# naver/deep-image-retrieval

Hardware: AMD Instinct MI355X
Metric: images/sec descriptor extraction (resnet101-GeM, 1024x1024) (higher is better)
Workload: dtype fp16p

## Files before the change

### deep-image-retrieval_amd/csrc/engine.hip

```cpp
#include "engine.h"

#include <math.h>
#include <algorithm>

namespace dir {

static thread_local std::string g_err;
void set_error(const std::string& msg) { g_err = msg; }
int fail(int code, const std::string& msg) {
    g_err = msg;
    return code;
}
const char* last_error() { return g_err.c_str(); }


static Env read_env() {
    Env e;
    auto on = [](const char* k) { return getenv(k) != nullptr; };
    const char* mode = getenv("DIRTORCH_AMD_C3C1");
    e.c3c1_off = mode && mode[0] == '0';
    e.c3c1_force = mode && mode[0] == 'f';
    e.no_ds_seam = on("DIRTORCH_AMD_NO_DS_SEAM");
    e.no_dual = on("DIRTORCH_AMD_NO_DUAL");
    e.rev_conv1 = on("DIRTORCH_AMD_REV_CONV1");
// ... 379 lines not shown

int dir_engine::overflow(hipStream_t stream, int* overflowed) {
    if (!finalized) return fail(DIR_ERR_STATE, "overflow query before finalize");
    int host = 0;
    DIR_HIP_CHECK(hipMemcpyAsync(&host, d_ovf, sizeof(int), hipMemcpyDeviceToHost, stream));
    DIR_HIP_CHECK(hipMemsetAsync(d_ovf, 0, sizeof(int), stream));
    DIR_HIP_CHECK(hipStreamSynchronize(stream));
    *overflowed = host != 0;
    return DIR_OK;
}

static inline int conv_out(int h, int k, int stride, int pad) { return (h + 2 * pad - k) / stride + 1; }

int dir_engine::plan(int B, int H, int W, Plan* p) const {
    if (B <= 0 || H <= 0 || W <= 0) return fail(DIR_ERR_INVALID, "forward: B, H, W must be positive");
    if (H < 7 || W < 7) return fail(DIR_ERR_INVALID, "forward: image smaller than the 7x7 stem");
    p->H2 = (H + 1) / 2;
    p->W2 = (W + 1) / 2;
    p->OH1 = conv_out(H, 7, 2, 3);
    p->OW1 = conv_out(W, 7, 2, 3);
    p->PH = conv_out(p->OH1, 3, 2, 1);
    p->PW = conv_out(p->OW1, 3, 2, 1);
    const size_t es = dtype == DIR_F32 ? 4 : 2;
    size_t io = 0, t1 = 0, t2 = 0, ds = 0, x4 = 0;
    int h = p->PH, w = p->PW;
    io = (size_t)B * h * w * 64 * es;
    for (size_t bi = 0; bi < blocks.size(); ++bi) {
        const BlockDef& bd = blocks[bi];
        const int oh = conv_out(h, 3, bd.stride, 1), ow = conv_out(w, 3, bd.stride, 1);
        const ConvLayer& c1 = convs[bd.conv1];
        const ConvLayer& cl = convs[desc.bottleneck ? bd.conv3 : bd.conv2];
        if (desc.bottleneck) {
            t1 = std::max(t1, (size_t)B * h * w * c1.Cout * es);
            t2 = std::max(t2, (size_t)B * oh * ow * convs[bd.conv2].Cout * es);
        } else {
            t1 = std::max(t1, (size_t)B * oh * ow * c1.Cout * es);
        }
        if (bd.down >= 0) ds = std::max(ds, (size_t)B * oh * ow * convs[bd.down].Cout * es);
        io = std::max(io, (size_t)B * oh * ow * cl.Cout * es);
        h = oh;
        w = ow;
        if ((int)bi == x4_block) {
            x4 = (size_t)B * h * w * x4_dim * es;
            t2 = std::max(t2, x4);
        }
    }
    if (conv1x5 >= 0) t1 = std::max(t1, (size_t)B * h * w * x4_dim * es);
    size_t off = 0;
    auto take = [&](size_t bytes) {
        const size_t o = off;
        off += align_up(bytes);
        return o;
    };
    p->s2d = take((size_t)B * p->H2 * p->W2 * 16 * es);
    p->stem = take((size_t)B * p->OH1 * p->OW1 * 64 * es);
    p->bufA = take(io);
    p->bufB = take(io);
    p->t1 = take(t1);
    p->t2 = take(t2 ? t2 : 256);
    p->ds = take(ds ? ds : 256);
    p->x4 = take(x4 ? x4 : 256);
    p->lo_s2d = p->lo_stem = p->lo_t1 = p->lo_t2 = p->lo_ds = 0;
    if (dtype == DIR_FP16P) {
        size_t pt1 = 0, pt2 = 0, pds = 0;
        int ph = p->PH, pw = p->PW;
        for (int bi = 0; pair_acts && bi < pair_blocks && bi < (int)blocks.size(); ++bi) {
            const BlockDef& bd = blocks[bi];
            const int oh = conv_out(ph, 3, bd.stride, 1), ow = conv_out(pw, 3, bd.stride, 1);
            const ConvLayer& c1 = convs[bd.conv1];
            if (desc.bottleneck) {
                pt1 = std::max(pt1, (size_t)B * ph * pw * c1.Cout * 2);
                pt2 = std::max(pt2, (size_t)B * oh * ow * convs[bd.conv2].Cout * 2);
            } else {
                pt1 = std::max(pt1, (size_t)B * oh * ow * c1.Cout * 2);
            }
            if (bd.down >= 0) pds = std::max(pds, (size_t)B * oh * ow * convs[bd.down].Cout * 2);
            ph = oh;
            pw = ow;
        }
        p->lo_s2d = take((size_t)B * p->H2 * p->W2 * 16 * 2);
        p->lo_stem = take((size_t)B * p->PH * p->PW * 64 * 2);
        p->lo_t1 = take(pt1 ? pt1 : 256);
        p->lo_t2 = take(pt2 ? pt2 : 256);
        p->lo_ds = take(pds ? pds : 256);
    }
    p->splitk = take(kSplitKMaxBytes);
    p->pooled = take((size_t)B * head_dim * 4);
    p->fcout = take((size_t)B * std::max(desc.out_dim, head_dim) * 4);
    p->total = off;
    return DIR_OK;
}

int dir_engine::prof_begin(const std::string& name, const std::string& kernel, double flops,
                           double bytes, hipStream_t stream) {
    if (!profiling || prof_paused) return DIR_OK;
    if (prof_used == prof.size()) {
        ProfSlot s;
        DIR_HIP_CHECK(hipEventCreate(&s.start));
        DIR_HIP_CHECK(hipEventCreate(&s.stop));
        prof.push_back(s);
    }
    ProfSlot& s = prof[prof_used];
    s.name = name;
    s.kernel = kernel;
    s.flops = flops;
    s.bytes = bytes;
    DIR_HIP_CHECK(hipEventRecord(s.start, stream));
// ... 113 lines not shown
    a.x_lo = x_lo;
    a.w = L.d_w;
    a.w_lo = L.d_w_lo;
    a.bias = L.d_bias;
    a.res = res;
    a.res_lo = res_lo;
    a.y = y;
    a.y_lo = y_lo;
    a.B = B;
    a.H = H;
    a.W = W;
    a.OH = OH;
    a.OW = OW;
    a.Cin = L.Cin;
    a.Cout = L.Cout;
    a.R = L.R;
    a.S = L.S;
    a.stride = L.stride;
    a.pad = L.pad;
    a.relu = L.relu ? 1 : 0;
    a.ovf = d_ovf;
    a.M = B * OH * OW;
    a.Ktot = a.R * a.S * a.Cin;
    if (x2) {
        a.x2 = x2;
        a.x2_lo = x2_lo;
        a.Cin2 = a.Cin;
        a.w = L.d_w_ds;
        a.w_lo = L.d_w_ds_lo;
        a.bias = L.d_bias_ds;
        a.Ktot = 2 * a.Cin;
    }
    const double macs = (double)a.M * L.Cout * (double)a.Ktot;
    const double bytes = 2.0 * ((double)B * H * W * a.Cin * (x_lo ? 2 : 1) * (x2 ? 2 : 1) + (double)a.M * L.Cout * (y_lo ? 2 : 1) +
                                (double)a.M * L.Cout * (res ? (res_lo ? 2 : 1) : 0) + 2.0 * L.Cout * a.Ktot);
    int rc = DIR_OK;
    if (profiling && !prof_paused)
        rc = prof_begin(x2 ? L.name.substr(0, L.name.rfind('.')) + ".ds+conv3" : L.name,
                        std::string("conv_pair<") + conv_pair_variant_name(a) + ">", 2.0 * macs, bytes, stream);
    if (rc != DIR_OK) return rc;
    rc = conv_pair_launch(a, stream);
    if (rc != DIR_OK) return rc;
    return prof_end(stream);
}

int dir_engine::forward_pair_stem(const void* img, int B, int H, int W, int fmt, char* base, const Plan& p,
                                  hipStream_t stream) {
    uint16_t* s2d = (uint16_t*)(base + p.s2d);
    uint16_t* s2d_lo = (uint16_t*)(base + p.lo_s2d);
    int rc;
    if (img && fmt == DIR_IMG_U8_NHWC && d_stem_u8_w && !sw.no_stem_u8) {
        const bool raw = stem_pool_u8_raw_ok(img, B, H, W);
        if (!raw) {
            rc = prof_begin("prep_input", "prep_input_u8", 0, (double)B * H * W * 3 + (double)B * p.H2 * p.W2 * 32, stream);
            if (rc != DIR_OK) return rc;
            rc = prep_input_u8(img, s2d, B, H, W, stream);
            if (rc != DIR_OK) return rc;
            if ((rc = prof_end(stream)) != DIR_OK) return rc;
        }
        rc = prof_begin("conv1+maxpool", "stem_pool_u8", 2.0 * B * p.OH1 * p.OW1 * 64.0 * 147.0,
                        (raw ? (double)B * H * W * 3 : 2.0 * (double)B * p.H2 * p.W2 * 16) + 4.0 * ((double)B * p.PH * p.PW * 64 + 64 * 256),
                        stream);
        if (rc != DIR_OK) return rc;
        rc = stem_pool_u8_launch(raw ? img : nullptr, s2d, d_stem_u8_w, d_stem_u8_w_lo, d_stem_u8_bias, d_stem_u8_corr,
                                 (uint16_t*)(base + p.bufA), (uint16_t*)(base + p.lo_stem), B, H, W, stream, d_ovf, sw.stem_u8_seg);
        if (rc != DIR_OK) return rc;
        return prof_end(stream);
    }
    const bool raw_f32 = img && fmt == DIR_IMG_F32_NCHW && stem_pool_pair_raw_ok(img, B, H, W);
    if (img && !raw_f32) {
        rc = prof_begin("prep_input", "prep_input_pair", 0, (double)B * H * W * 3 * (fmt == DIR_IMG_U8_NHWC ? 1 : 4) +
                        (double)B * p.H2 * p.W2 * 64, stream);
        if (rc != DIR_OK) return rc;
        rc = prep_input_pair(img, fmt, desc.mean, desc.std, s2d, s2d_lo, B, H, W, stream);
        if (rc != DIR_OK) return rc;
        if ((rc = prof_end(stream)) != DIR_OK) return rc;
    } else if (!img) {
        const long n = (long)B * p.H2 * p.W2 * 16;
        hipLaunchKernelGGL(fill_noise_kernel, dim3((unsigned)((n + 255) / 256)), dim3(256), 0, stream, s2d, n, DIR_FP16);
        DIR_HIP_CHECK(hipGetLastError());
        DIR_HIP_CHECK(hipMemsetAsync(s2d_lo, 0, (size_t)n * 2, stream));
    }
    rc = prof_begin("conv1+maxpool", "stem_pool_pair", 2.0 * B * p.OH1 * p.OW1 * 64.0 * 147.0,
                    (raw_f32 ? (double)B * H * W * 12 : 4.0 * (double)B * p.H2 * p.W2 * 16) + 4.0 * ((double)B * p.PH * p.PW * 64 + 64 * 256), stream);
    if (rc != DIR_OK) return rc;
    if (raw_f32)
        rc = stem_pool_pair_walk_launch(nullptr, nullptr, convs[0].d_w, convs[0].d_w_lo, convs[0].d_bias, (uint16_t*)(base + p.bufA),
                                        (uint16_t*)(base + p.lo_stem), B, p.H2, p.W2, p.OH1, p.OW1, stream, d_ovf, img, H, W);
    else
        rc = stem_pool_pair_launch(s2d, s2d_lo, convs[0].d_w, convs[0].d_w_lo, convs[0].d_bias, (uint16_t*)(base + p.bufA),
                                   (uint16_t*)(base + p.lo_stem), B, p.H2, p.W2, p.OH1, p.OW1, stream, d_ovf);
    if (rc != DIR_OK) return rc;
    return prof_end(stream);
}

int dir_engine::forward_pair_head(const void* img, int B, int H, int W, int fmt, char* base, const Plan& p,
                                  hipStream_t stream, uint16_t** cur_out, int* h_out, int* w_out, size_t* next_block) {
    uint16_t* const pp[2] = {(uint16_t*)(base + p.bufA), (uint16_t*)(base + p.bufB)};
    uint16_t* stem_lo = (uint16_t*)(base + p.lo_stem);
    uint16_t* t1 = (uint16_t*)(base + p.t1);
    uint16_t* t2 = (uint16_t*)(base + p.t2);
    uint16_t* ds = (uint16_t*)(base + p.ds);
    uint16_t* t1_lo = (uint16_t*)(base + p.lo_t1);
    uint16_t* t2_lo = (uint16_t*)(base + p.lo_t2);
    uint16_t* ds_lo = (uint16_t*)(base + p.lo_ds);
    int rc = forward_pair_stem(img, B, H, W, fmt, base, p, stream);
    if (rc != DIR_OK) return rc;
    int cur = 0;

    int h = p.PH, w = p.PW;
    const size_t nb = std::min((size_t)pair_blocks, blocks.size());
    for (size_t bi = 0; bi < nb; ++bi) {
        BlockDef& bd = blocks[bi];
        const int oh = conv_out(h, 3, bd.stride, 1), ow = conv_out(w, 3, bd.stride, 1);
// ... 528 lines not shown
```

### deep-image-retrieval_amd/csrc/stem_u8.hip

```cpp
#include "dir_common.h"
#include "conv_igemm.h"
#include "pointwise.h"

#include <math.h>
#include <stdio.h>
#include <stdlib.h>
#include <vector>

#ifndef DIR_STEMU8_ABL
#define DIR_STEMU8_ABL 0
#endif

namespace dir {

static constexpr uint32_t kOOBu = 0x80000000u;

__device__ __forceinline__ void dma16u(__amdgpu_buffer_rsrc_t rsrc, char* lds, uint32_t voff) {
    __builtin_amdgcn_raw_ptr_buffer_load_lds(rsrc, (DIR_LDS void*)lds, 16, voff, 0, 0, 0);
}
__device__ __forceinline__ void split2u(float a, float b, uint32_t& hi, uint32_t& lo) {
    hi = FP16::pack(a, b);
    float ha, hb;
    FP16::unpack(hi, ha, hb);
    lo = FP16::pack(a - ha, b - hb);
// ... 14 lines not shown
    const float* bias;
    const float* corr;
    uint16_t *yh, *yl;
    int B, H, W, H2, W2, OH, OW, PH, PW;
    int tiles_x, nseg, seg_rows, nitems;
    uint32_t x_bytes;
    int* ovf;
};

struct TileU8 {
    int valid;
    int item, t, nt;
    int b, pw0;
    int pbase, pe;
    int c;
};

__device__ __forceinline__ int border_class(int o, int n) {
    const int t = 2 * o + 4 - n;
    return o == 0 ? 1 : (o == 1 ? 2 : (t <= 0 ? 0 : 2 + t));
}

template <int NRP, bool RAW, bool XPAIR = false>
__global__ void __launch_bounds__(128 * NRP, NRP == 2 ? 2 : 1) stem_pool_u8_kernel(const StemU8Args a) {
    typedef FP16 DT;
    typedef DT::frag_t frag_t;
    constexpr int PTW = 15;
    constexpr int NT = 128 * NRP;
    constexpr int TH = 2 * NRP, TW = 32;
    constexpr int QW = TW + 3;
    constexpr int QP = (TH + 3) * QW;
    constexpr int PLANE = NT * 16;
    constexpr int PATCH = (XPAIR ? 4 : 2) * PLANE;
    constexpr int NPB = XPAIR ? 2 : 3;
    constexpr int XROW = 16 * 256;
    constexpr int XBUF = 2 * NRP * XROW;
    static_assert(QP <= NT, "one DMA instruction per plane covers the patch");
    constexpr int X_OFF = NPB * PATCH;
    constexpr int BIAS_OFF = X_OFF + 2 * XBUF;
    constexpr int CORR_OFF = BIAS_OFF + 256;

    extern __shared__ __attribute__((aligned(16))) char smem[];

    const int tid = threadIdx.x;
    const int lane = tid & 63;
    const int wave = __builtin_amdgcn_readfirstlane(tid >> 6);
    const int lrow = lane & 31, lhi = lane >> 5;
    const int ci = wave & 1, rp = wave >> 1;

    const __amdgpu_buffer_rsrc_t rsrc_x = RAW ? __builtin_amdgcn_make_buffer_rsrc((void*)a.img, 0, a.img_bytes, 0x00020000)
                                              : __builtin_amdgcn_make_buffer_rsrc((void*)a.x, 0, a.x_bytes, 0x00020000);
    const __amdgpu_buffer_rsrc_t rsrc_xl = __builtin_amdgcn_make_buffer_rsrc((void*)(XPAIR ? a.xl : a.x), 0, a.x_bytes, 0x00020000);

    frag_t wfh[4][4], wfl[4][4];
#pragma unroll
    for (int R = 0; R < 4; ++R)
#pragma unroll
        for (int ks = 0; ks < 4; ++ks) {
            const size_t o = (size_t)(ci * 32 + lrow) * 256 + R * 64 + ks * 16 + lhi * 8;
            wfh[R][ks] = __builtin_bit_cast(frag_t, gload16(a.wh + o));
            wfl[R][ks] = __builtin_bit_cast(frag_t, gload16(a.wl + o));
        }
    float* lbias = (float*)(smem + BIAS_OFF);
    float* lcorr = (float*)(smem + CORR_OFF);
    if (tid < 64) lbias[tid] = a.bias[tid];
    if (!XPAIR)
        for (int i = tid; i < 36 * 64; i += NT) lcorr[i] = a.corr[i];

    auto decode = [&](TileU8& d) {
        d.valid = d.item < a.nitems;
        if (!d.valid) return;
        int r = d.item;
        const int tx = r % a.tiles_x;
        r /= a.tiles_x;
        d.b = r % a.B;
        const int seg = r / a.B;
        const int ps = seg * a.seg_rows;
        d.pe = min(a.PH, ps + a.seg_rows);
        d.nt = (2 * (d.pe - ps) + TH) / TH;
        d.pw0 = tx * PTW;
        d.pbase = ps + NRP * d.t;
        d.c = 2 * ps - 1 + TH * d.t;
    };
    auto advance = [&](TileU8& d) {
        if (!d.valid) return;
        if (++d.t < d.nt) {
            d.pbase += NRP;
            d.c += TH;
        } else {
            d.item += gridDim.x;
            d.t = 0;
            decode(d);
        }
    };
    const int ppy = tid / QW, ppx = tid - ppy * QW;
    const int ppoff = (ppy * a.W2 + ppx) * 32;
    auto issue_patch = [&](const TileU8& d, char* dst) {
        const int iy = d.c - 2 + ppy, ix = 2 * d.pw0 - 3 + ppx;
        const bool ok = tid < QP && (unsigned)iy < (unsigned)a.H2 && (unsigned)ix < (unsigned)a.W2;
        const int base = ((d.b * a.H2 + d.c - 2) * a.W2 + 2 * d.pw0 - 3) * 32;
        const uint32_t v = ok ? (uint32_t)(base + ppoff) : kOOBu;
        if (DIR_STEMU8_ABL & 4) return;
        dma16u(rsrc_x, dst + (wave * 64) * 16, v);
        dma16u(rsrc_x, dst + (NT + wave * 64) * 16, ok ? v + 16 : kOOBu);
        if (XPAIR) {
            dma16u(rsrc_xl, dst + (2 * NT + wave * 64) * 16, v);
            dma16u(rsrc_xl, dst + (3 * NT + wave * 64) * 16, ok ? v + 16 : kOOBu);
        }
    };

    uint32_t rw[XPAIR ? 12 : 6] = {};
    auto load_raw = [&](const TileU8& d) {
        const int iy = d.c - 2 + ppy, ix = 2 * d.pw0 - 3 + ppx;
        const bool ok = tid < QP && (unsigned)iy < (unsigned)a.H2 && (unsigned)ix < (unsigned)a.W2;
        if (XPAIR) {
            const int plane = a.H * a.W;
            const uint32_t o0 = ok ? (uint32_t)((((d.b * 3) * a.H + 2 * iy) * a.W + 2 * ix) * 4) : kOOBu;
            const bool row1 = ok && 2 * iy + 1 < a.H;
#pragma unroll
            for (int c = 0; c < 3; ++c)
#pragma unroll
                for (int dy = 0; dy < 2; ++dy) {
                    const uint32_t o = (dy == 0 ? ok : row1) ? o0 + (uint32_t)((c * plane + dy * a.W) * 4) : kOOBu;
                    const u32x2_t v = __builtin_bit_cast(u32x2_t, __builtin_amdgcn_raw_buffer_load_b64(rsrc_x, o, 0, 0));
                    rw[(c * 2 + dy) * 2] = v[0];
                    rw[(c * 2 + dy) * 2 + 1] = v[1];
                }
            return;
        }
        const uint32_t o0 = ok ? (uint32_t)(((d.b * a.H + 2 * iy) * a.W + 2 * ix) * 3) : kOOBu;
        const uint32_t o1 = (ok && 2 * iy + 1 < a.H) ? o0 + (uint32_t)(a.W * 3) : kOOBu;
#pragma unroll
        for (int k = 0; k < 3; ++k) {
            rw[k] = __builtin_amdgcn_raw_buffer_load_b16(rsrc_x, o0 + 2 * k, 0, 0);
            rw[3 + k] = __builtin_amdgcn_raw_buffer_load_b16(rsrc_x, o1 + 2 * k, 0, 0);
        }
    };
    auto store_raw = [&](char* dst) {
        if (XPAIR) {
            float f[12];
#pragma unroll
            for (int c = 0; c < 3; ++c)
#pragma unroll
                for (int dy = 0; dy < 2; ++dy)
#pragma unroll
                    for (int dx = 0; dx < 2; ++dx) f[(dy * 2 + dx) * 3 + c] = __builtin_bit_cast(float, rw[(c * 2 + dy) * 2 + dx]);
            u32x4_t h0, h1, l0, l1;
#pragma unroll
            for (int e = 0; e < 4; ++e) {
                uint32_t hh, ll;
                split2u(f[2 * e], f[2 * e + 1], hh, ll);
                h0[e] = hh;
                l0[e] = ll;
            }
#pragma unroll
            for (int e = 0; e < 2; ++e) {
                uint32_t hh, ll;
                split2u(f[8 + 2 * e], f[9 + 2 * e], hh, ll);
                h1[e] = hh;
                l1[e] = ll;
            }
            h1[2] = h1[3] = l1[2] = l1[3] = 0;
            *(u32x4_t*)(dst + tid * 16) = h0;
            *(u32x4_t*)(dst + (NT + tid) * 16) = h1;
            *(u32x4_t*)(dst + (2 * NT + tid) * 16) = l0;
            *(u32x4_t*)(dst + (3 * NT + tid) * 16) = l1;
            return;
        }
        float f[12];
#pragma unroll
        for (int k = 0; k < 6; ++k) {
            f[2 * k] = (float)(rw[k] & 0xffu) * 0.00390625f;
            f[2 * k + 1] = (float)((rw[k] >> 8) & 0xffu) * 0.00390625f;
        }
        u32x4_t p0, p1;
#pragma unroll
        for (int e = 0; e < 4; ++e) p0[e] = FP16::pack(f[2 * e], f[2 * e + 1]);
        p1[0] = FP16::pack(f[8], f[9]);
        p1[1] = FP16::pack(f[10], f[11]);
        p1[2] = p1[3] = 0;
        *(u32x4_t*)(dst + tid * 16) = p0;
        *(u32x4_t*)(dst + (NT + tid) * 16) = p1;
    };

    TileU8 cur, nxt, pre, prev;
    cur.item = blockIdx.x;
    cur.t = 0;
    decode(cur);
    if (!cur.valid) return;
    nxt = cur;
    advance(nxt);
    pre = nxt;
    advance(pre);
    prev.valid = 0;
    prev.t = prev.b = prev.pw0 = prev.pbase = prev.pe = 0;

    Ovf<DT> ovf;
    asm volatile("s_waitcnt vmcnt(0) lgkmcnt(0)" ::: "memory");
#pragma unroll
    for (int R = 0; R < 4; ++R)
#pragma unroll
        for (int ks = 0; ks < 4; ++ks) {
            asm volatile("" : "+v"(wfh[R][ks]));
            asm volatile("" : "+v"(wfl[R][ks]));
        }
    if (RAW) {
        load_raw(cur);
        store_raw(smem);
        if (nxt.valid) load_raw(nxt);
    } else {
        issue_patch(cur, smem);
        if (!XPAIR && nxt.valid) issue_patch(nxt, smem + PATCH);
    }

    int pb = 0;
    int xb = 0;
    for (;;) {
        if (RAW)
            asm volatile("s_waitcnt lgkmcnt(0)" ::: "memory");
        else if (XPAIR)
            asm volatile("s_waitcnt vmcnt(0) lgkmcnt(0)" ::: "memory");
        else if (nxt.valid)
            asm volatile("s_waitcnt vmcnt(2) lgkmcnt(0)" ::: "memory");
        else
            asm volatile("s_waitcnt vmcnt(0) lgkmcnt(0)" ::: "memory");
        ring_barrier();

        if (RAW) {
            if (nxt.valid) store_raw(smem + (pb == NPB - 1 ? 0 : pb + 1) * PATCH);
            if (pre.valid) load_raw(pre);
        } else if (XPAIR) {
            if (nxt.valid) issue_patch(nxt, smem + (pb ^ 1) * PATCH);
        } else if (pre.valid) {
            const int nb = pb == 0 ? 2 : pb - 1;
            issue_patch(pre, smem + nb * PATCH);
        }

        if (prev.valid && !(DIR_STEMU8_ABL & 2)) {
            const char* X = smem + X_OFF + (xb ^ 1) * XBUF;
            const int r4 = tid >> 7, px = (tid >> 3) & 15, c8 = tid & 7;
            const int ph = r4 < NRP - 1 ? prev.pbase + r4 : prev.pbase - 1;
            const int pw = prev.pw0 + px;
            const bool live = px < PTW && pw < a.PW && ph < prev.pe && (r4 < NRP - 1 || prev.t > 0);
            if (live) {
                const int o0 = px * 256 + (((2 * c8) ^ (px & 7)) << 4), o1 = px * 256 + (((2 * c8 + 1) ^ (px & 7)) << 4);
                f32x4_t m0, m1;
                if (r4 < NRP - 1) {
                    const f32x4_t a0 = *(const f32x4_t*)(X + r4 * XROW + o0), a1 = *(const f32x4_t*)(X + r4 * XROW + o1);
                    const f32x4_t b0 = *(const f32x4_t*)(X + (NRP + r4) * XROW + o0), b1 = *(const f32x4_t*)(X + (NRP + r4) * XROW + o1);
#pragma unroll
                    for (int e = 0; e < 4; ++e) {
                        m0[e] = fmaxf(a0[e], b0[e]);
                        m1[e] = fmaxf(a1[e], b1[e]);
                    }
                } else {
                    m0 = *(const f32x4_t*)(X + (2 * NRP - 1) * XROW + o0);
                    m1 = *(const f32x4_t*)(X + (2 * NRP - 1) * XROW + o1);
                }
                f32x4_t bb0 = {0.f, 0.f, 0.f, 0.f}, bb1 = {0.f, 0.f, 0.f, 0.f};
                if (!XPAIR) {
                    bb0 = *(const f32x4_t*)(lbias + c8 * 8);
                    bb1 = *(const f32x4_t*)(lbias + c8 * 8 + 4);
                }
                u32x4_t oh, ol;
                float mv[8];
#pragma unroll
                for (int e = 0; e < 4; ++e) {
                    mv[e] = fmaxf(XPAIR ? m0[e] : m0[e] + bb0[e], 0.f);
                    mv[4 + e] = fmaxf(XPAIR ? m1[e] : m1[e] + bb1[e], 0.f);
                }
#pragma unroll
                for (int e = 0; e < 4; ++e) {
                    uint32_t hh, ll;
                    split2u(mv[2 * e], mv[2 * e + 1], hh, ll);
                    oh[e] = hh;
                    ol[e] = ll;
                }
                const size_t o = ((size_t)(prev.b * a.PH + ph) * a.PW + pw) * 64 + c8 * 8;
                gstore16(a.yh + o, oh);
                gstore16(a.yl + o, ol);
                ovf.see(oh);
            }
        }
        if (!cur.valid) break;

        const char* pbuf = smem + pb * PATCH;
        const int ox = 2 * cur.pw0 - 1 + lrow;
        const int oy = cur.c + 2 * rp;
        const bool edge = cur.c <= 1 || 2 * (cur.c + TH - 1) + 4 > a.H || cur.pw0 == 0 || 2 * (2 * cur.pw0 + TW - 2) + 4 > a.W;
        f32x16_t acc[2];
        if (XPAIR) {
#pragma unroll
            for (int g = 0; g < 4; ++g) {
                const f32x4_t b4 = *(const f32x4_t*)(lbias + ci * 32 + 8 * g + 4 * lhi);
#pragma unroll
                for (int j = 0; j < 2; ++j)
#pragma unroll
                    for (int e = 0; e < 4; ++e) acc[j][4 * g + e] = b4[e];
            }
        } else {
#pragma unroll
            for (int j = 0; j < 2; ++j)
#pragma unroll
                for (int e = 0; e < 16; ++e) acc[j][e] = 0.f;
        }
        const char* xrow = pbuf + lhi * PLANE + ((rp * 2) * QW + lrow) * 16;
        frag_t xf[2], xg[2];
        xf[0] = *(const frag_t*)xrow;
        if (XPAIR) xg[0] = *(const frag_t*)(xrow + 2 * PLANE);
#pragma unroll
        for (int s = 0; s < 20; ++s) {
            const int q = s >> 2, ks = s & 3;
            if (s + 1 < 20) {
                xf[(s + 1) & 1] = *(const frag_t*)(xrow + (((s + 1) >> 2) * QW + ((s + 1) & 3)) * 16);
                if (XPAIR) xg[(s + 1) & 1] = *(const frag_t*)(xrow + 2 * PLANE + (((s + 1) >> 2) * QW + ((s + 1) & 3)) * 16);
            }
            if (!(DIR_STEMU8_ABL & 1)) {
                if (q < 4) {
                    acc[0] = DT::mfma32(wfh[q][ks], xf[s & 1], acc[0]);
                    if (XPAIR) acc[0] = DT::mfma32(wfh[q][ks], xg[s & 1], acc[0]);
                    acc[0] = DT::mfma32(wfl[q][ks], xf[s & 1], acc[0]);
                }
                if (q > 0) {
                    acc[1] = DT::mfma32(wfh[q - 1][ks], xf[s & 1], acc[1]);
                    if (XPAIR) acc[1] = DT::mfma32(wfh[q - 1][ks], xg[s & 1], acc[1]);
                    acc[1] = DT::mfma32(wfl[q - 1][ks], xf[s & 1], acc[1]);
                }
            }
            if (XPAIR) continue;
            __builtin_amdgcn_sched_group_barrier(0x100, 1, 0);
            if (q > 0 && q < 4)
                __builtin_amdgcn_sched_group_barrier(0x008, 4, 0);
            else
                __builtin_amdgcn_sched_group_barrier(0x008, 2, 0);
        }

        if (edge) {
            const bool col_in = (unsigned)ox < (unsigned)a.OW;
            const int cc = XPAIR ? 0 : border_class(min(max(ox, 0), a.OW - 1), a.W);
#pragma unroll
            for (int j = 0; j < 2; ++j) {
                const bool in = col_in && (unsigned)(oy + j) < (unsigned)a.OH;
                const int rc = XPAIR ? 0 : border_class(min(max(oy + j, 0), a.OH - 1), a.H);
#pragma unroll
                for (int g = 0; g < 4; ++g) {
                    f32x4_t c4 = {0.f, 0.f, 0.f, 0.f};
                    if (!XPAIR) c4 = *(const f32x4_t*)(lcorr + (rc * 6 + cc) * 64 + ci * 32 + 8 * g + 4 * lhi);
#pragma unroll
                    for (int e = 0; e < 4; ++e) {
                        const float t = acc[j][4 * g + e];
                        acc[j][4 * g + e] = in ? t + c4[e] : -__builtin_inff();
                    }
                }
            }
        }
#pragma unroll
        for (int j = 0; j < 2; ++j)
#pragma unroll
            for (int e = 0; e < 16; ++e) {
                const float v = acc[j][e];
                acc[j][e] = fmaxf(fmaxf(lane_left(v), v), lane_right(v));
            }
        char* X = smem + X_OFF + xb * XBUF;
        const int px = lrow >> 1;
        const bool odd = (lrow & 1) != 0;
        if (rp == 0 && cur.t > 0) {
            const char* Xp = smem + X_OFF + (xb ^ 1) * XBUF;
            if (odd) {
#pragma unroll
                for (int g = 0; g < 4; ++g) {
                    const int off = px * 256 + (((8 * ci + 2 * g + lhi) ^ (px & 7)) << 4);
                    const f32x4_t m3 = *(const f32x4_t*)(Xp + (NRP - 1) * XROW + off);
                    f32x4_t v;
#pragma unroll
                    for (int e = 0; e < 4; ++e) v[e] = fmaxf(m3[e], acc[0][4 * g + e]);
                    *(f32x4_t*)(X + (2 * NRP - 1) * XROW + off) = v;
                }
            }
        }
        if (odd) {
#pragma unroll
            for (int g = 0; g < 4; ++g) {
                const int off = px * 256 + (((8 * ci + 2 * g + lhi) ^ (px & 7)) << 4);
                f32x4_t h, m;
#pragma unroll
                for (int e = 0; e < 4; ++e) {
                    h[e] = acc[0][4 * g + e];
                    m[e] = fmaxf(acc[0][4 * g + e], acc[1][4 * g + e]);
                }
                *(f32x4_t*)(X + rp * XROW + off) = m;
                if (rp > 0) *(f32x4_t*)(X + (NRP - 1 + rp) * XROW + off) = h;
            }
        }

        prev = cur;
        cur = nxt;
        nxt = pre;
        advance(pre);
        pb = pb == NPB - 1 ? 0 : pb + 1;
        xb ^= 1;
    }
    ovf.flush(a.ovf);
}

__global__ void __launch_bounds__(256) prep_input_u8_kernel(const uint8_t* __restrict__ img, uint16_t* __restrict__ out, int B, int H,
                                                            int W, int H2, int W2) {
    const long idx = (long)blockIdx.x * blockDim.x + threadIdx.x;
    const long total = (long)B * H2 * W2;
    if (idx >= total) return;
    const int x2 = (int)(idx % W2);
    const int y2 = (int)((idx / W2) % H2);
    const int b = (int)(idx / ((long)W2 * H2));
    float v[16];
#pragma unroll
    for (int e = 0; e < 16; ++e) v[e] = 0.f;
#pragma unroll
    for (int dy = 0; dy < 2; ++dy) {
        const int y = 2 * y2 + dy;
        if (y >= H) continue;
        const uint8_t* row = img + (((size_t)b * H + y) * W + 2 * x2) * 3;
        const int n = (2 * x2 + 1 < W) ? 6 : 3;
#pragma unroll
        for (int k = 0; k < 6; ++k)
            if (k < n) v[dy * 6 + k] = (float)row[k] * 0.00390625f;
    }
    u32x4_t o0, o1;
#pragma unroll
    for (int e = 0; e < 4; ++e) {
        o0[e] = FP16::pack(v[2 * e], v[2 * e + 1]);
        o1[e] = FP16::pack(v[8 + 2 * e], v[8 + 2 * e + 1]);
    }
    gstore16(out + idx * 16, o0);
    gstore16(out + idx * 16 + 8, o1);
}

int fold_stem_u8(const float* w, const float* scale, const float* bias, const float* mean3, const float* std3,
                 std::vector<uint16_t>& hi, std::vector<uint16_t>& lo, std::vector<float>& b2, std::vector<float>& corr) {
    for (int c = 0; c < 3; ++c)
        if (!(std3[c] > 0.f)) return fail(DIR_ERR_INVALID, "stem_u8: preprocess std must be positive");
    const int lo_r[6] = {0, 3, 1, 0, 0, 0}, hi_r[6] = {6, 6, 6, 5, 4, 3};
    std::vector<float> packed((size_t)64 * 256, 0.f);
    b2.assign(64, 0.f);
    corr.assign((size_t)36 * 64, 0.f);
    for (int o = 0; o < 64; ++o) {
        double all = 0.0;
        double in[6][6];
        for (int rc = 0; rc < 6; ++rc)
            for (int cc = 0; cc < 6; ++cc) in[rc][cc] = 0.0;
        for (int c = 0; c < 3; ++c) {
            const double ms = (double)mean3[c] / (double)std3[c];
            for (int r = 0; r < 7; ++r)
                for (int s = 0; s < 7; ++s) {
                    const double ws = (double)w[(((size_t)o * 3 + c) * 7 + r) * 7 + s] * (double)scale[o];
                    all += ws * ms;
                    for (int rc = 0; rc < 6; ++rc)
                        for (int cc = 0; cc < 6; ++cc)
                            if (r >= lo_r[rc] && r <= hi_r[rc] && s >= lo_r[cc] && s <= hi_r[cc]) in[rc][cc] += ws * ms;
                    const int R = (r + 1) >> 1, dy = (r + 1) & 1, S = (s + 1) >> 1, dx = (s + 1) & 1;
                    packed[(((size_t)o * 4 + R) * 4 + S) * 16 + (dy * 2 + dx) * 3 + c] = (float)(ws * 256.0 / (255.0 * (double)std3[c]));
                }
        }
        b2[o] = (float)((double)bias[o] - all);
        for (int rc = 0; rc < 6; ++rc)
            for (int cc = 0; cc < 6; ++cc) corr[((size_t)rc * 6 + cc) * 64 + o] = (float)(all - in[rc][cc]);
    }
    hi.resize(packed.size());
    lo.resize(packed.size());
    for (size_t i = 0; i < packed.size(); ++i) {
        hi[i] = f32_to_f16_bits(packed[i]);
        if ((hi[i] & 0x7c00u) == 0x7c00u && std::isfinite(packed[i]))
            return fail(DIR_ERR_RANGE, "finalize: a BatchNorm-folded weight of conv1, folded with the image normalisation (" + std::to_string(packed[i]) +
                                           ") exceeds the fp16 range; use DIR_BF16 or DIR_F32");
        lo[i] = f32_to_f16_bits(packed[i] - f16_bits_to_f32(hi[i]));
    }
    return DIR_OK;
}

int prep_input_u8(const void* img, void* out, int B, int H, int W, hipStream_t stream) {
    if (!img || !out) return fail(DIR_ERR_INVALID, "prep_input_u8: null pointer");
    const int H2 = (H + 1) / 2, W2 = (W + 1) / 2;
    const long total = (long)B * H2 * W2;
    hipLaunchKernelGGL(prep_input_u8_kernel, dim3((unsigned)((total + 255) / 256)), dim3(256), 0, stream, (const uint8_t*)img,
                       (uint16_t*)out, B, H, W, H2, W2);
    DIR_HIP_CHECK(hipGetLastError());
    return DIR_OK;
}

bool stem_pool_u8_raw_ok(const void* img, int B, int H, int W) {
    return img && (W % 2) == 0 && ((uintptr_t)img & 1) == 0 && (size_t)B * H * W * 3 < (1ull << 31) && !env().stem_u8_prep &&
           !env().stem_u8_wg8;
}

int stem_pool_u8_launch(const void* img, const void* s2d, const void* w_hi, const void* w_lo, const float* bias, const float* corr,
                        void* y_hi, void* y_lo, int B, int H, int W, hipStream_t stream, int* ovf, int seg_tiles) {
    const bool raw = stem_pool_u8_raw_ok(img, B, H, W);
    if ((!raw && !s2d) || !w_hi || !w_lo || !bias || !corr || !y_hi || !y_lo) return fail(DIR_ERR_INVALID, "stem_pool_u8: null pointer");
    if (H < 7 || W < 7) return fail(DIR_ERR_INVALID, "stem_pool_u8: image smaller than the 7x7 stem");
    StemU8Args a;
    a.img = (const uint8_t*)img;
    a.img_bytes = raw ? (uint32_t)((size_t)B * H * W * 3) : 0;
    a.x = (const uint16_t*)s2d;
    a.xl = nullptr;
    a.wh = (const uint16_t*)w_hi;
    a.wl = (const uint16_t*)w_lo;
    a.bias = bias;
    a.corr = corr;
    a.yh = (uint16_t*)y_hi;
    a.yl = (uint16_t*)y_lo;
    a.B = B; a.H = H; a.W = W;
    a.H2 = (H + 1) / 2;
    a.W2 = (W + 1) / 2;
    a.OH = (H - 1) / 2 + 1;
    a.OW = (W - 1) / 2 + 1;
    a.PH = (a.OH - 1) / 2 + 1;
    a.PW = (a.OW - 1) / 2 + 1;
    if (!raw && (size_t)B * a.H2 * a.W2 * 32 >= (1ull << 31))
        return fail(DIR_ERR_INVALID, "stem_pool_u8: input exceeds 2^31 bytes; lower the batch");
    a.x_bytes = raw ? 0 : (uint32_t)((size_t)B * a.H2 * a.W2 * 32);
    a.tiles_x = (a.PW + 14) / 15;
    const bool wg8 = env().stem_u8_wg8;
    const int cus = cu_count();
    const int slots = wg8 ? cus : 2 * cus;
    int T = seg_tiles > 0 ? seg_tiles : 8;
    while (seg_tiles <= 0 && T > 1 && (long)B * a.tiles_x * ((a.PH + 4 * T - 2) / (4 * T - 1)) < 2L * slots) T >>= 1;
    a.seg_rows = 4 * T - 1;
    a.nseg = (a.PH + a.seg_rows - 1) / a.seg_rows;
    a.nitems = B * a.tiles_x * a.nseg;
    a.ovf = ovf;
    const int grid = a.nitems < slots ? a.nitems : slots;
    if (wg8) {
        constexpr int LDS = 3 * 16384 + 2 * 8 * 4096 + 256 + 36 * 64 * 4;
        static std::atomic<uint64_t> attr{0};
        DIR_HIP_CHECK(ensure_dynamic_lds((const void*)(stem_pool_u8_kernel<4, false>), LDS, attr));
        hipLaunchKernelGGL((stem_pool_u8_kernel<4, false>), dim3((unsigned)grid), dim3(512), LDS, stream, a);
    } else {
        constexpr int LDS = 3 * 8192 + 2 * 4 * 4096 + 256 + 36 * 64 * 4;
        static std::atomic<uint64_t> attr{0};
        static std::atomic<uint64_t> attr_raw{0};
        DIR_HIP_CHECK(ensure_dynamic_lds((const void*)(stem_pool_u8_kernel<2, false>), LDS, attr));
        DIR_HIP_CHECK(ensure_dynamic_lds((const void*)(stem_pool_u8_kernel<2, true>), LDS, attr_raw));
        static const bool dbg = getenv("DIRTORCH_AMD_DEBUG_OCCUPANCY") != nullptr;
        static std::atomic<int> told{0};
        if (dbg && !told.exchange(1)) {
            int nb = -1;
            (void)hipOccupancyMaxActiveBlocksPerMultiprocessor(&nb, (const void*)(stem_pool_u8_kernel<2, true>), 256, LDS);
            fprintf(stderr, "stem_pool_u8_kernel<2>: %d workgroups of 256 threads per CU at %d bytes of LDS (grid %d, %d items)\n", nb, LDS, grid,
                    a.nitems);
        }
        if (raw)
            hipLaunchKernelGGL((stem_pool_u8_kernel<2, true>), dim3((unsigned)grid), dim3(256), LDS, stream, a);
        else
            hipLaunchKernelGGL((stem_pool_u8_kernel<2, false>), dim3((unsigned)grid), dim3(256), LDS, stream, a);
    }
    DIR_HIP_CHECK(hipGetLastError());
    return DIR_OK;
}

bool stem_pool_pair_raw_ok(const void* img_f32, int B, int H, int W) {
    return img_f32 && (W % 2) == 0 && ((uintptr_t)img_f32 & 7) == 0 && (size_t)B * 3 * H * W * 4 < (1ull << 31) && !env().stem_u8_prep &&
           !env().stem_pair_old && !env().stem_v1;
}

int stem_pool_pair_walk_launch(const void* s2d_hi, const void* s2d_lo, const void* w_hi, const void* w_lo, const float* bias,
                               void* y_hi, void* y_lo, int B, int H2, int W2, int OH, int OW, hipStream_t stream, int* ovf,
                               const void* img_f32, int H, int W) {
    const bool raw = stem_pool_pair_raw_ok(img_f32, B, H, W);
    if ((!raw && (!s2d_hi || !s2d_lo)) || !w_hi || !w_lo || !bias || !y_hi || !y_lo) return fail(DIR_ERR_INVALID, "stem_pool_pair: null pointer");
    if (!raw && (size_t)B * H2 * W2 * 32 >= (1ull << 31)) return fail(DIR_ERR_INVALID, "stem_pool_pair: input exceeds 2^31 bytes; lower the batch");
    StemU8Args a;
    a.img = (const uint8_t*)(raw ? img_f32 : nullptr);
    a.img_bytes = raw ? (uint32_t)((size_t)B * 3 * H * W * 4) : 0;
// ... 39 lines not shown
```

### deep-image-retrieval_amd/dirtorch_amd/ops.py

```python
import ctypes

import torch

from . import _lib
from ._lib import DIR_BF16, DIR_FP16, POOLING, call, ptr, stream_ptr


def _dtype_code(t):
    if t.dtype == torch.bfloat16:
        return DIR_BF16
    if t.dtype == torch.float16:
        return DIR_FP16
    raise TypeError('16-bit activation tensor expected (bfloat16 or float16), got %s' % t.dtype)


def _need_cuda(*ts):
    for t in ts:
        if t is not None and not t.is_cuda:
            raise ValueError('device tensor expected')
        if t is not None and not t.is_contiguous():
            raise ValueError('contiguous tensor expected')


def conv_variant_names():
# ... 331 lines not shown
    y_hi = torch.empty(B, H, W, Cout, dtype=torch.float16, device=t_hi.device)
    y_lo = torch.empty_like(y_hi) if pair_out else None
    call('dir_conv_pair_dual', ptr(t_hi), ptr(t_lo), ptr(x_hi), ptr(x_lo), ptr(w_hi), ptr(w_lo), ptr(bias), ptr(y_hi),
         ptr(y_lo), B, H, W, Cin, Cout, int(bool(relu)), stream_ptr())
    return y_hi, y_lo


def prep_input_pair(img, mean=None, std=None):
    _need_cuda(img)
    if img.dtype == torch.float32:
        B, C, H, W = img.shape
        fmt = _lib.DIR_IMG_F32_NCHW
    elif img.dtype == torch.uint8:
        B, H, W, C = img.shape
        fmt = _lib.DIR_IMG_U8_NHWC
    else:
        raise TypeError('image must be float32 NCHW or uint8 NHWC')
    if C != 3:
        raise ValueError('3-channel image expected')
    hi = torch.empty(B, (H + 1) // 2, (W + 1) // 2, 16, dtype=torch.float16, device=img.device)
    lo = torch.empty_like(hi)
    m = (ctypes.c_float * 3)(*(mean or (0, 0, 0)))
    s = (ctypes.c_float * 3)(*(std or (1, 1, 1)))
    call('dir_prep_input_pair', ptr(img), fmt, m, s, ptr(hi), ptr(lo), B, H, W, stream_ptr())
    return hi, lo


def stem_pool_pair(s2d, w_packed, bias, out_hw):
    (s_hi, s_lo), (w_hi, w_lo) = s2d, w_packed
    _need_cuda(s_hi, s_lo, w_hi, w_lo, bias)
    B, H2, W2, _ = s_hi.shape
    OH, OW = out_hw
    PH, PW = (OH - 1) // 2 + 1, (OW - 1) // 2 + 1
    y_hi = torch.empty(B, PH, PW, 64, dtype=torch.float16, device=s_hi.device)
    y_lo = torch.empty_like(y_hi)
    call('dir_stem_pool_pair', ptr(s_hi), ptr(s_lo), ptr(w_hi), ptr(w_lo), ptr(bias), ptr(y_hi), ptr(y_lo), B, H2, W2,
         OH, OW, stream_ptr())
    return y_hi, y_lo


def stem_pool_u8(img_u8, w_oihw, bn_scale, bn_bias, mean, std, seg_tiles=0):
    _need_cuda(img_u8)
    if img_u8.dtype != torch.uint8 or img_u8.dim() != 4 or img_u8.shape[3] != 3:
        raise TypeError('image must be uint8 NHWC [B,H,W,3]')
    B, H, W, _ = img_u8.shape
    OH, OW = (H - 1) // 2 + 1, (W - 1) // 2 + 1
    PH, PW = (OH - 1) // 2 + 1, (OW - 1) // 2 + 1
    w = w_oihw.detach().to('cpu', torch.float32).contiguous()
    sc = bn_scale.detach().to('cpu', torch.float32).contiguous()
    bi = bn_bias.detach().to('cpu', torch.float32).contiguous()
    assert tuple(w.shape) == (64, 3, 7, 7) and sc.numel() == 64 and bi.numel() == 64
    m = (ctypes.c_float * 3)(*mean)
    s = (ctypes.c_float * 3)(*std)
    ws = torch.empty(B * ((H + 1) // 2) * ((W + 1) // 2) * 32, dtype=torch.uint8, device=img_u8.device)
    y_hi = torch.empty(B, PH, PW, 64, dtype=torch.float16, device=img_u8.device)
    y_lo = torch.empty_like(y_hi)
    call('dir_stem_pool_u8', ptr(img_u8.contiguous()), ctypes.c_void_p(w.data_ptr()), ctypes.c_void_p(sc.data_ptr()),
         ctypes.c_void_p(bi.data_ptr()), m, s, ptr(ws), ptr(y_hi), ptr(y_lo), B, H, W, int(seg_tiles), stream_ptr())
    return y_hi, y_lo


def pca_whiten(X, components, mean=None, alpha=None, l2norm=False, eps_unused=None, unit_range=False):
    _need_cuda(X, components, mean, alpha)
    for t in (X, components, mean, alpha):
        if t is not None and (t.dtype != torch.float32 or not t.is_contiguous()):
            raise TypeError('contiguous float32 tensors expected')
    N, D = X.shape
    v, D2 = components.shape
    if D != D2:
        raise ValueError('inner dimensions differ')
    out = torch.empty(N, v, dtype=torch.float32, device=X.device)
    if N == 0:
        return out
    call('dir_pca_whiten_l2_unit' if unit_range else 'dir_pca_whiten_l2', ptr(X), N, D, ptr(mean), ptr(components), v, ptr(alpha),
         int(bool(l2norm)), ptr(out), stream_ptr())
    return out
```

Baseline: 2467.

## Repack u8 stem input so conv1 K-dimension uses three MFMA slices instead of four

The space-to-depth layout for the uint8 stem now packs the 12 real channels per 2x2 cell so that the 7x7 conv reduction uses three 16-wide K slices per row instead of four zero-padded ones. The input buffer gains one extra padded column, the prep kernel and raw loader write shifted/overlapping halves, and the weight packing is reorganised to match. This cuts MFMA count and weight registers in the stem by about a quarter, at the cost of more complex indexing, a slightly larger staging buffer and extra LDS writes in the raw path.

```diff
diff --git a/deep-image-retrieval_amd/csrc/engine.hip b/deep-image-retrieval_amd/csrc/engine.hip
--- a/deep-image-retrieval_amd/csrc/engine.hip
+++ b/deep-image-retrieval_amd/csrc/engine.hip
@@ -455,7 +455,7 @@
         off += align_up(bytes);
         return o;
     };
-    p->s2d = take((size_t)B * p->H2 * p->W2 * 16 * es);
+    p->s2d = take((size_t)B * p->H2 * (p->W2 + (dtype == DIR_FP16P ? 1 : 0)) * 16 * es);
     p->stem = take((size_t)B * p->OH1 * p->OW1 * 64 * es);
     p->bufA = take(io);
     p->bufB = take(io);
@@ -675,14 +675,14 @@
     if (img && fmt == DIR_IMG_U8_NHWC && d_stem_u8_w && !sw.no_stem_u8) {
         const bool raw = stem_pool_u8_raw_ok(img, B, H, W);
         if (!raw) {
-            rc = prof_begin("prep_input", "prep_input_u8", 0, (double)B * H * W * 3 + (double)B * p.H2 * p.W2 * 32, stream);
+            rc = prof_begin("prep_input", "prep_input_u8", 0, (double)B * H * W * 3 + (double)B * p.H2 * (p.W2 + 1) * 32, stream);
             if (rc != DIR_OK) return rc;
             rc = prep_input_u8(img, s2d, B, H, W, stream);
             if (rc != DIR_OK) return rc;
             if ((rc = prof_end(stream)) != DIR_OK) return rc;
         }
         rc = prof_begin("conv1+maxpool", "stem_pool_u8", 2.0 * B * p.OH1 * p.OW1 * 64.0 * 147.0,
-                        (raw ? (double)B * H * W * 3 : 2.0 * (double)B * p.H2 * p.W2 * 16) + 4.0 * ((double)B * p.PH * p.PW * 64 + 64 * 256),
+                        (raw ? (double)B * H * W * 3 : 2.0 * (double)B * p.H2 * (p.W2 + 1) * 16) + 4.0 * ((double)B * p.PH * p.PW * 64 + 64 * 192),
                         stream);
         if (rc != DIR_OK) return rc;
         rc = stem_pool_u8_launch(raw ? img : nullptr, s2d, d_stem_u8_w, d_stem_u8_w_lo, d_stem_u8_bias, d_stem_u8_corr,
diff --git a/deep-image-retrieval_amd/csrc/stem_u8.hip b/deep-image-retrieval_amd/csrc/stem_u8.hip
--- a/deep-image-retrieval_amd/csrc/stem_u8.hip
+++ b/deep-image-retrieval_amd/csrc/stem_u8.hip
@@ -90,12 +90,13 @@
                                               : __builtin_amdgcn_make_buffer_rsrc((void*)a.x, 0, a.x_bytes, 0x00020000);
     const __amdgpu_buffer_rsrc_t rsrc_xl = __builtin_amdgcn_make_buffer_rsrc((void*)(XPAIR ? a.xl : a.x), 0, a.x_bytes, 0x00020000);
 
-    frag_t wfh[4][4], wfl[4][4];
+    constexpr int KS = XPAIR ? 4 : 3;
+    frag_t wfh[4][KS], wfl[4][KS];
 #pragma unroll
     for (int R = 0; R < 4; ++R)
 #pragma unroll
-        for (int ks = 0; ks < 4; ++ks) {
-            const size_t o = (size_t)(ci * 32 + lrow) * 256 + R * 64 + ks * 16 + lhi * 8;
+        for (int ks = 0; ks < KS; ++ks) {
+            const size_t o = (size_t)(ci * 32 + lrow) * (64 * KS) + R * (16 * KS) + ks * 16 + lhi * 8;
             wfh[R][ks] = __builtin_bit_cast(frag_t, gload16(a.wh + o));
             wfl[R][ks] = __builtin_bit_cast(frag_t, gload16(a.wl + o));
         }
@@ -132,11 +133,12 @@
         }
     };
     const int ppy = tid / QW, ppx = tid - ppy * QW;
-    const int ppoff = (ppy * a.W2 + ppx) * 32;
+    const int xw = XPAIR ? a.W2 : a.W2 + 1, xs = XPAIR ? 0 : 1;
+    const int ppoff = (ppy * xw + ppx) * 32;
     auto issue_patch = [&](const TileU8& d, char* dst) {
         const int iy = d.c - 2 + ppy, ix = 2 * d.pw0 - 3 + ppx;
-        const bool ok = tid < QP && (unsigned)iy < (unsigned)a.H2 && (unsigned)ix < (unsigned)a.W2;
-        const int base = ((d.b * a.H2 + d.c - 2) * a.W2 + 2 * d.pw0 - 3) * 32;
+        const bool ok = tid < QP && (unsigned)iy < (unsigned)a.H2 && (unsigned)(ix + xs) < (unsigned)xw;
+        const int base = ((d.b * a.H2 + d.c - 2) * xw + 2 * d.pw0 - 3 + xs) * 32;
         const uint32_t v = ok ? (uint32_t)(base + ppoff) : kOOBu;
         if (DIR_STEMU8_ABL & 4) return;
         dma16u(rsrc_x, dst + (wave * 64) * 16, v);
@@ -151,6 +153,7 @@
     auto load_raw = [&](const TileU8& d) {
         const int iy = d.c - 2 + ppy, ix = 2 * d.pw0 - 3 + ppx;
         const bool ok = tid < QP && (unsigned)iy < (unsigned)a.H2 && (unsigned)ix < (unsigned)a.W2;
+        if (DIR_STEMU8_ABL & 4) return;
         if (XPAIR) {
             const int plane = a.H * a.W;
             const uint32_t o0 = ok ? (uint32_t)((((d.b * 3) * a.H + 2 * iy) * a.W + 2 * ix) * 4) : kOOBu;
@@ -211,14 +214,15 @@
             f[2 * k] = (float)(rw[k] & 0xffu) * 0.00390625f;
             f[2 * k + 1] = (float)((rw[k] >> 8) & 0xffu) * 0.00390625f;
         }
-        u32x4_t p0, p1;
+        u32x4_t p0;
+        u32x2_t p1;
 #pragma unroll
         for (int e = 0; e < 4; ++e) p0[e] = FP16::pack(f[2 * e], f[2 * e + 1]);
         p1[0] = FP16::pack(f[8], f[9]);
         p1[1] = FP16::pack(f[10], f[11]);
-        p1[2] = p1[3] = 0;
         *(u32x4_t*)(dst + tid * 16) = p0;
-        *(u32x4_t*)(dst + (NT + tid) * 16) = p1;
+        *(u32x2_t*)(dst + (NT + tid) * 16) = p1;
+        if (ppx > 0) *(u32x2_t*)(dst + (NT + tid - 1) * 16 + 8) = p1;
     };
 
     TileU8 cur, nxt, pre, prev;
@@ -238,7 +242,7 @@
 #pragma unroll
     for (int R = 0; R < 4; ++R)
 #pragma unroll
-        for (int ks = 0; ks < 4; ++ks) {
+        for (int ks = 0; ks < KS; ++ks) {
             asm volatile("" : "+v"(wfh[R][ks]));
             asm volatile("" : "+v"(wfl[R][ks]));
         }
@@ -342,35 +346,60 @@
 #pragma unroll
                 for (int e = 0; e < 16; ++e) acc[j][e] = 0.f;
         }
-        const char* xrow = pbuf + lhi * PLANE + ((rp * 2) * QW + lrow) * 16;
-        frag_t xf[2], xg[2];
-        xf[0] = *(const frag_t*)xrow;
-        if (XPAIR) xg[0] = *(const frag_t*)(xrow + 2 * PLANE);
-#pragma unroll
-        for (int s = 0; s < 20; ++s) {
-            const int q = s >> 2, ks = s & 3;
-            if (s + 1 < 20) {
-                xf[(s + 1) & 1] = *(const frag_t*)(xrow + (((s + 1) >> 2) * QW + ((s + 1) & 3)) * 16);
-                if (XPAIR) xg[(s + 1) & 1] = *(const frag_t*)(xrow + 2 * PLANE + (((s + 1) >> 2) * QW + ((s + 1) & 3)) * 16);
-            }
-            if (!(DIR_STEMU8_ABL & 1)) {
-                if (q < 4) {
-                    acc[0] = DT::mfma32(wfh[q][ks], xf[s & 1], acc[0]);
-                    if (XPAIR) acc[0] = DT::mfma32(wfh[q][ks], xg[s & 1], acc[0]);
-                    acc[0] = DT::mfma32(wfl[q][ks], xf[s & 1], acc[0]);
-                }
-                if (q > 0) {
-                    acc[1] = DT::mfma32(wfh[q - 1][ks], xf[s & 1], acc[1]);
-                    if (XPAIR) acc[1] = DT::mfma32(wfh[q - 1][ks], xg[s & 1], acc[1]);
-                    acc[1] = DT::mfma32(wfl[q - 1][ks], xf[s & 1], acc[1]);
-                }
-            }
-            if (XPAIR) continue;
-            __builtin_amdgcn_sched_group_barrier(0x100, 1, 0);
-            if (q > 0 && q < 4)
-                __builtin_amdgcn_sched_group_barrier(0x008, 4, 0);
-            else
-                __builtin_amdgcn_sched_group_barrier(0x008, 2, 0);
+        if constexpr (XPAIR) {
+            const char* xrow = pbuf + lhi * PLANE + ((rp * 2) * QW + lrow) * 16;
+            frag_t xf[2], xg[2];
+            xf[0] = *(const frag_t*)xrow;
+            xg[0] = *(const frag_t*)(xrow + 2 * PLANE);
+#pragma unroll
+            for (int s = 0; s < 20; ++s) {
+                const int q = s >> 2, ks = s & 3;
+                if (s + 1 < 20) {
+                    xf[(s + 1) & 1] = *(const frag_t*)(xrow + (((s + 1) >> 2) * QW + ((s + 1) & 3)) * 16);
+                    xg[(s + 1) & 1] = *(const frag_t*)(xrow + 2 * PLANE + (((s + 1) >> 2) * QW + ((s + 1) & 3)) * 16);
+                }
+                if (!(DIR_STEMU8_ABL & 1)) {
+                    if (q < 4) {
+                        acc[0] = DT::mfma32(wfh[q][ks], xf[s & 1], acc[0]);
+                        acc[0] = DT::mfma32(wfh[q][ks], xg[s & 1], acc[0]);
+                        acc[0] = DT::mfma32(wfl[q][ks], xf[s & 1], acc[0]);
+                    }
+                    if (q > 0) {
+                        acc[1] = DT::mfma32(wfh[q - 1][ks], xf[s & 1], acc[1]);
+                        acc[1] = DT::mfma32(wfh[q - 1][ks], xg[s & 1], acc[1]);
+                        acc[1] = DT::mfma32(wfl[q - 1][ks], xf[s & 1], acc[1]);
+                    }
+                }
+            }
+        } else {
+            const char* xa = pbuf + ((rp * 2) * QW + lrow + lhi) * 16;
+            const char* xb2 = pbuf + PLANE + ((rp * 2) * QW + lrow + 2 * lhi) * 16;
+            auto frag = [&](int s) {
+                const int q = s / 3, sl = s - 3 * q;
+                return *(const frag_t*)(sl == 2 ? xb2 + q * QW * 16 : xa + (q * QW + 2 * sl) * 16);
+            };
+            frag_t xf[2];
+            xf[0] = frag(0);
+#pragma unroll
+            for (int s = 0; s < 15; ++s) {
+                const int q = s / 3, ks = s - 3 * q;
+                if (s + 1 < 15) xf[(s + 1) & 1] = frag(s + 1);
+                if (!(DIR_STEMU8_ABL & 1)) {
+                    if (q < 4) {
+                        acc[0] = DT::mfma32(wfh[q][ks], xf[s & 1], acc[0]);
+                        acc[0] = DT::mfma32(wfl[q][ks], xf[s & 1], acc[0]);
+                    }
+                    if (q > 0) {
+                        acc[1] = DT::mfma32(wfh[q - 1][ks], xf[s & 1], acc[1]);
+                        acc[1] = DT::mfma32(wfl[q - 1][ks], xf[s & 1], acc[1]);
+                    }
+                }
+                __builtin_amdgcn_sched_group_barrier(0x100, 1, 0);
+                if (q > 0 && q < 4)
+                    __builtin_amdgcn_sched_group_barrier(0x008, 4, 0);
+                else
+                    __builtin_amdgcn_sched_group_barrier(0x008, 2, 0);
+            }
         }
 
         if (edge) {
@@ -444,11 +473,11 @@
 __global__ void __launch_bounds__(256) prep_input_u8_kernel(const uint8_t* __restrict__ img, uint16_t* __restrict__ out, int B, int H,
                                                             int W, int H2, int W2) {
     const long idx = (long)blockIdx.x * blockDim.x + threadIdx.x;
-    const long total = (long)B * H2 * W2;
+    const long total = (long)B * H2 * (W2 + 1);
     if (idx >= total) return;
-    const int x2 = (int)(idx % W2);
-    const int y2 = (int)((idx / W2) % H2);
-    const int b = (int)(idx / ((long)W2 * H2));
+    const int x2 = (int)(idx % (W2 + 1)) - 1;
+    const int y2 = (int)((idx / (W2 + 1)) % H2);
+    const int b = (int)(idx / ((long)(W2 + 1) * H2));
     float v[16];
 #pragma unroll
     for (int e = 0; e < 16; ++e) v[e] = 0.f;
@@ -456,11 +485,19 @@
     for (int dy = 0; dy < 2; ++dy) {
         const int y = 2 * y2 + dy;
         if (y >= H) continue;
-        const uint8_t* row = img + (((size_t)b * H + y) * W + 2 * x2) * 3;
-        const int n = (2 * x2 + 1 < W) ? 6 : 3;
-#pragma unroll
-        for (int k = 0; k < 6; ++k)
-            if (k < n) v[dy * 6 + k] = (float)row[k] * 0.00390625f;
+        const uint8_t* row = img + (((size_t)b * H + y) * W) * 3;
+        if (x2 >= 0) {
+            const int n = (2 * x2 + 1 < W) ? 6 : 3;
+#pragma unroll
+            for (int k = 0; k < 6; ++k)
+                if (k < n) v[dy * 6 + k] = (float)row[(size_t)x2 * 6 + k] * 0.00390625f;
+        }
+        if (dy == 1 && x2 + 1 < W2) {
+            const int n = (2 * x2 + 3 < W) ? 6 : 3;
+#pragma unroll
+            for (int k = 2; k < 6; ++k)
+                if (k < n) v[10 + k] = (float)row[(size_t)(x2 + 1) * 6 + k] * 0.00390625f;
+        }
     }
     u32x4_t o0, o1;
 #pragma unroll
@@ -477,7 +514,7 @@
     for (int c = 0; c < 3; ++c)
         if (!(std3[c] > 0.f)) return fail(DIR_ERR_INVALID, "stem_u8: preprocess std must be positive");
     const int lo_r[6] = {0, 3, 1, 0, 0, 0}, hi_r[6] = {6, 6, 6, 5, 4, 3};
-    std::vector<float> packed((size_t)64 * 256, 0.f);
+    std::vector<float> packed((size_t)64 * 192, 0.f);
     b2.assign(64, 0.f);
     corr.assign((size_t)36 * 64, 0.f);
     for (int o = 0; o < 64; ++o) {
@@ -495,7 +532,9 @@
                         for (int cc = 0; cc < 6; ++cc)
                             if (r >= lo_r[rc] && r <= hi_r[rc] && s >= lo_r[cc] && s <= hi_r[cc]) in[rc][cc] += ws * ms;
                     const int R = (r + 1) >> 1, dy = (r + 1) & 1, S = (s + 1) >> 1, dx = (s + 1) & 1;
-                    packed[(((size_t)o * 4 + R) * 4 + S) * 16 + (dy * 2 + dx) * 3 + c] = (float)(ws * 256.0 / (255.0 * (double)std3[c]));
+                    const int ch = (dy * 2 + dx) * 3 + c;
+                    const int slice = ch < 8 ? S >> 1 : 2, k = ch < 8 ? 8 * (S & 1) + ch : 4 * S + ch - 8;
+                    packed[(((size_t)o * 4 + R) * 3 + slice) * 16 + k] = (float)(ws * 256.0 / (255.0 * (double)std3[c]));
                 }
         }
         b2[o] = (float)((double)bias[o] - all);
@@ -517,7 +556,7 @@
 int prep_input_u8(const void* img, void* out, int B, int H, int W, hipStream_t stream) {
     if (!img || !out) return fail(DIR_ERR_INVALID, "prep_input_u8: null pointer");
     const int H2 = (H + 1) / 2, W2 = (W + 1) / 2;
-    const long total = (long)B * H2 * W2;
+    const long total = (long)B * H2 * (W2 + 1);
     hipLaunchKernelGGL(prep_input_u8_kernel, dim3((unsigned)((total + 255) / 256)), dim3(256), 0, stream, (const uint8_t*)img,
                        (uint16_t*)out, B, H, W, H2, W2);
     DIR_HIP_CHECK(hipGetLastError());
@@ -552,9 +591,9 @@
     a.OW = (W - 1) / 2 + 1;
     a.PH = (a.OH - 1) / 2 + 1;
     a.PW = (a.OW - 1) / 2 + 1;
-    if (!raw && (size_t)B * a.H2 * a.W2 * 32 >= (1ull << 31))
+    if (!raw && (size_t)B * a.H2 * (a.W2 + 1) * 32 >= (1ull << 31))
         return fail(DIR_ERR_INVALID, "stem_pool_u8: input exceeds 2^31 bytes; lower the batch");
-    a.x_bytes = raw ? 0 : (uint32_t)((size_t)B * a.H2 * a.W2 * 32);
+    a.x_bytes = raw ? 0 : (uint32_t)((size_t)B * a.H2 * (a.W2 + 1) * 32);
     a.tiles_x = (a.PW + 14) / 15;
     const bool wg8 = env().stem_u8_wg8;
     const int cus = cu_count();
diff --git a/deep-image-retrieval_amd/dirtorch_amd/ops.py b/deep-image-retrieval_amd/dirtorch_amd/ops.py
--- a/deep-image-retrieval_amd/dirtorch_amd/ops.py
+++ b/deep-image-retrieval_amd/dirtorch_amd/ops.py
@@ -407,7 +407,7 @@
     assert tuple(w.shape) == (64, 3, 7, 7) and sc.numel() == 64 and bi.numel() == 64
     m = (ctypes.c_float * 3)(*mean)
     s = (ctypes.c_float * 3)(*std)
-    ws = torch.empty(B * ((H + 1) // 2) * ((W + 1) // 2) * 32, dtype=torch.uint8, device=img_u8.device)
+    ws = torch.empty(B * ((H + 1) // 2) * ((W + 1) // 2 + 1) * 32, dtype=torch.uint8, device=img_u8.device)
     y_hi = torch.empty(B, PH, PW, 64, dtype=torch.float16, device=img_u8.device)
     y_lo = torch.empty_like(y_hi)
     call('dir_stem_pool_u8', ptr(img_u8.contiguous()), ctypes.c_void_p(w.data_ptr()), ctypes.c_void_p(sc.data_ptr()),
```

New measurement: 2476 (median of 6 runs). No clear change (+0.4%).
